# ethnhe/FFB6D

Measured on AMD Instinct MI355X. Metric: RGB-D frames/sec fwd (480x640, N=12288, bs=8), higher is better.
Workload: dtype f32; 1 GPU; FFB6D forward incl. on-device 22-call KNN index pyramid; bs=8/GPU, N=12288 pts, 480x640 RGB-D, 22 classes, fp32, eval; global_batch=8, n_points=12288, index_dtype=int64, layout=pm, parallelism=dp1 (independent batches, one process per GPU, no process group)

## Files before the change

### ffb6d_amd/csrc/mfma_pm.h

```cpp
#pragma once
#include <hip/hip_runtime.h>

namespace ffb6d {
namespace pm {

typedef float f32x16 __attribute__((ext_vector_type(16)));
typedef unsigned int u32x4 __attribute__((ext_vector_type(4)));
typedef __bf16 bf16x8 __attribute__((ext_vector_type(8)));

constexpr int BLK = 256;

template <typename T> struct El;
template <> struct El<float> {
    static constexpr int SZ = 4;
    typedef float4 Raw4;
    static __device__ __forceinline__ Raw4 ld4raw(const float* p) { return *reinterpret_cast<const float4*>(p); }
    static __device__ __forceinline__ float4 cvt4(Raw4 r) { return r; }
    static __device__ __forceinline__ float4 ld4(const float* p) { return *reinterpret_cast<const float4*>(p); }
    static __device__ __forceinline__ void st4(float* p, float4 v) { *reinterpret_cast<float4*>(p) = v; }
    static __device__ __forceinline__ float ld(const float* p) { return *p; }
    static __device__ __forceinline__ void st(float* p, float v) { *p = v; }
};
template <> struct El<__bf16> {
    static constexpr int SZ = 2;
    typedef uint2 Raw4;
    static __device__ __forceinline__ Raw4 ld4raw(const __bf16* p) { return *reinterpret_cast<const uint2*>(p); }
    static __device__ __forceinline__ float4 cvt4(Raw4 u)
    {
        return make_float4(__uint_as_float(u.x << 16), __uint_as_float(u.x & 0xffff0000u), __uint_as_float(u.y << 16),
                           __uint_as_float(u.y & 0xffff0000u));
    }
    static __device__ __forceinline__ float4 ld4(const __bf16* p) { return cvt4(ld4raw(p)); }
    static __device__ __forceinline__ void st4(__bf16* p, float4 v)
    {
        typedef __bf16 bf16x4 __attribute__((ext_vector_type(4)));
        const bf16x4 b = {(__bf16)v.x, (__bf16)v.y, (__bf16)v.z, (__bf16)v.w};
        *reinterpret_cast<bf16x4*>(p) = b;
    }
    static __device__ __forceinline__ float ld(const __bf16* p) { return (float)*p; }
    static __device__ __forceinline__ void st(__bf16* p, float v) { *p = (__bf16)v; }
};

template <typename T, int TM, int TN>
__device__ __forceinline__ void mfma_step(f32x16 (&acc)[TM][TN], const u32x4 (&a)[TM], const u32x4 (&b)[TN])
{
    if constexpr (El<T>::SZ == 4) {
#pragma unroll
        for (int tt = 0; tt < 4; ++tt)
#pragma unroll
            for (int i = 0; i < TM; ++i)
#pragma unroll
                for (int j = 0; j < TN; ++j)
                    acc[i][j] = __builtin_amdgcn_mfma_f32_32x32x2f32(__uint_as_float(a[i][tt]), __uint_as_float(b[j][tt]),
                                                                     acc[i][j], 0, 0, 0);
    } else {
#pragma unroll
        for (int i = 0; i < TM; ++i)
#pragma unroll
            for (int j = 0; j < TN; ++j)
                acc[i][j] = __builtin_amdgcn_mfma_f32_32x32x16_bf16(__builtin_bit_cast(bf16x8, a[i]), __builtin_bit_cast(bf16x8, b[j]),
                                                                    acc[i][j], 0, 0, 0);
    }
}

typedef float f32x4 __attribute__((ext_vector_type(4)));
__device__ __forceinline__ f32x4 mfma_16x16x4(float a, float b, f32x4 c)
{
#if __has_builtin(__builtin_amdgcn_mfma_f32_16x16x4f32)
    return __builtin_amdgcn_mfma_f32_16x16x4f32(a, b, c, 0, 0, 0);
#else
    const int l = (int)(threadIdx.x & 63u);
    for (int k = 0; k < 4; ++k) {
        const float bk = __shfl(b, 16 * k + (l & 15), 64);
        for (int r = 0; r < 4; ++r) c[r] = fmaf(__shfl(a, 16 * k + 4 * (l >> 4) + r, 64), bk, c[r]);
    }
    return c;
#endif
}

__device__ __forceinline__ float activate(float v, float slope) { return fmaxf(v, slope * v); }

__device__ __forceinline__ __amdgpu_buffer_rsrc_t make_rsrc(const void* base, unsigned bytes)
{
    return __builtin_amdgcn_make_buffer_rsrc(const_cast<void*>(base), 0, bytes, 0x00020000);
}

__device__ __forceinline__ void lds_dma16(__amdgpu_buffer_rsrc_t rs, unsigned char* lds_dst, int voffset, int soffset)
{
    __builtin_amdgcn_raw_ptr_buffer_load_lds(rs, (__attribute__((address_space(3))) void*)lds_dst, 16, voffset, soffset, 0, 0);
}

template <int N>
__device__ __forceinline__ void lds_dma_wait()
{
    static_assert(N >= 0 && N < 64, "vmcnt is a 6-bit counter");
#if defined(__HIP_DEVICE_COMPILE__)
    __builtin_amdgcn_s_waitcnt((N & 15) | ((N >> 4) << 14) | 0x0F70);
#endif
}

__device__ __forceinline__ int opaque(int v)
{
#if defined(__HIP_DEVICE_COMPILE__)
    asm volatile("" : "+v"(v));
#endif
    return v;
}

__device__ __forceinline__ void use_here(unsigned v)
{
#if defined(__HIP_DEVICE_COMPILE__)
    asm volatile("" ::"v"(v));
#else
    (void)v;
#endif
}

}
}
```

### ffb6d_amd/csrc/mlp_pm_split.hip

```cpp
#include <algorithm>

#include "common.h"
#include "ffb6d_ops.h"
#include "mlp_pm_common.h"

namespace ffb6d {
namespace pm {
namespace {

constexpr int SP_BLK = 512;
constexpr int SP_RB = 64;
constexpr int SP_WIMG = 256 * SP_RB;
constexpr int SP_XIMG = 128 * SP_RB;
constexpr int SP_XBASE = 3 * SP_WIMG;
constexpr int SP_STAGE = 3 * SP_WIMG + 3 * SP_XIMG;
constexpr int SP_LDS = 2 * SP_STAGE;
static_assert(SP_LDS <= 160 * 1024, "LDS layout");

typedef __bf16 bf16x2 __attribute__((ext_vector_type(2)));

__device__ __forceinline__ void split3(float a, __bf16& a0, __bf16& a1, __bf16& a2)
{
    a0 = (__bf16)a;
    const float r1 = a - (float)a0;
    a1 = (__bf16)r1;
    a2 = (__bf16)(r1 - (float)a1);
}

__global__ void __launch_bounds__(256) split_w_kernel(const float* __restrict__ w, __bf16* __restrict__ w3, long long n)
{
    for (long long e = blockIdx.x * 256LL + threadIdx.x; e < n; e += 256LL * gridDim.x) {
        __bf16 a0, a1, a2;
        split3(w[e], a0, a1, a2);
        w3[e] = a0;
        w3[n + e] = a1;
        w3[2 * n + e] = a2;
    }
}

template <int VAR>
__global__ void __launch_bounds__(SP_BLK)
mlp_pm_split_kernel(const PmParams p, const unsigned part_bytes)
{
    constexpr int OOB = 0x7ffffff0;
    extern __shared__ __attribute__((aligned(16))) unsigned char lds[];

    const int t = blockIdx.x;
    const int xcd = t & 7, sl = t >> 3;
    const int pt = (sl / p.n_ct) * 8 + xcd;
    const int ct = sl % p.n_ct;
    if (pt >= p.n_pt) return;
    const int r0 = pt * 128, c0 = ct * 256;

    const int lane = threadIdx.x & 63;
    const int l31 = lane & 31, kh = lane >> 5;
    const int wave = __builtin_amdgcn_readfirstlane(threadIdx.x >> 6);
    const int wm = wave >> 2, wn = wave & 3;
    const int K = p.k1;
    const int nstep = K / 32;
    const int wrow0 = p.rows_per_w ? (r0 / p.rows_per_w) * p.cout : 0;

    const unsigned char* w3 = static_cast<const unsigned char*>(p.w);
    const __amdgpu_buffer_rsrc_t rs_w[3] = {make_rsrc(w3, part_bytes), make_rsrc(w3 + part_bytes, part_bytes),
                                            make_rsrc(w3 + 2 * (size_t)part_bytes, part_bytes)};
    const __amdgpu_buffer_rsrc_t rs_x = make_rsrc(p.x1, span_bytes((unsigned)p.rows, p.ld1, p.k1, 4));

    const int lrow = 16 * wave + (lane >> 2);
    const int lchunk = ((lane & 3) ^ ((lrow >> 3) & 3)) * 16;
    int w_off[2];
#pragma unroll
    for (int h = 0; h < 2; ++h) {
        const int ch = c0 + 128 * h + lrow;
        w_off[h] = ch < p.cout ? (wrow0 + ch) * (K * 2) + lchunk : OOB;
    }
    auto request_w = [&](int s, int stage) {
        unsigned char* wi = lds + stage * SP_STAGE + wave * (16 * SP_RB);
#pragma unroll
        for (int pi = 0; pi < 3; ++pi)
#pragma unroll
            for (int h = 0; h < 2; ++h) lds_dma16(rs_w[pi], wi + pi * SP_WIMG + h * (128 * SP_RB), w_off[h], s * SP_RB);
    };

    const int xrow = threadIdx.x >> 2, xq = threadIdx.x & 3;
    const bool xlive = r0 + xrow < p.rows;
    const int x_off0 = xlive ? (r0 + xrow) * p.ld1 * 4 + xq * 32 : OOB;
    const int x_off1 = xlive ? x_off0 + 16 : OOB;
    const int x_dst = SP_XBASE + xrow * SP_RB + ((xq ^ ((xrow >> 3) & 3)) * 16);
    auto load_x = [&](int s, u32x4 (&v)[2]) {
        v[0] = __builtin_amdgcn_raw_buffer_load_b128(rs_x, x_off0, s * 128, 0);
        v[1] = __builtin_amdgcn_raw_buffer_load_b128(rs_x, x_off1, s * 128, 0);
    };
    auto write_x = [&](int stage, const u32x4 (&v)[2]) {
        u32x4 o[3];
        if constexpr (VAR & 1) {
#pragma unroll
            for (int q = 0; q < 4; ++q) {
                const unsigned pk = (v[q >> 1][2 * (q & 1)] >> 16) | (v[q >> 1][2 * (q & 1) + 1] & 0xffff0000u);
                o[0][q] = pk; o[1][q] = 0u; o[2][q] = 0u;
            }
        } else {
#pragma unroll
            for (int q = 0; q < 4; ++q) {
                bf16x2 b0, b1, b2;
                __bf16 s0, s1, s2;
                split3(__uint_as_float(v[q >> 1][2 * (q & 1)]), s0, s1, s2);
                b0[0] = s0; b1[0] = s1; b2[0] = s2;
                split3(__uint_as_float(v[q >> 1][2 * (q & 1) + 1]), s0, s1, s2);
                b0[1] = s0; b1[1] = s1; b2[1] = s2;
                o[0][q] = __builtin_bit_cast(unsigned, b0);
                o[1][q] = __builtin_bit_cast(unsigned, b1);
                o[2][q] = __builtin_bit_cast(unsigned, b2);
            }
        }
        unsigned char* xi = lds + stage * SP_STAGE + x_dst;
#pragma unroll
        for (int pj = 0; pj < 3; ++pj) *reinterpret_cast<u32x4*>(xi + pj * SP_XIMG) = o[pj];
    };

    const int fsw = (l31 >> 3) & 3;
    const int a_row = (wm * 128 + l31) * SP_RB, b_row = SP_XBASE + (wn * 32 + l31) * SP_RB;
    f32x16 acc[4][1];
#pragma unroll
    for (int i = 0; i < 4; ++i)
#pragma unroll
        for (int r = 0; r < 16; ++r) acc[i][0][r] = 0.f;

    auto multiply = [&](int stage, int ks) {
        const unsigned char* im = lds + stage * SP_STAGE;
        const int fo = ((2 * ks + kh) ^ fsw) * 16;
        u32x4 a[3][4], b[3];
#pragma unroll
        for (int pj = 0; pj < 3; ++pj) b[pj] = *reinterpret_cast<const u32x4*>(im + b_row + pj * SP_XIMG + fo);
#pragma unroll
        for (int pi = 0; pi < 3; ++pi)
#pragma unroll
            for (int i = 0; i < 4; ++i) a[pi][i] = *reinterpret_cast<const u32x4*>(im + pi * SP_WIMG + a_row + i * (32 * SP_RB) + fo);
        if constexpr (VAR & 2) {
#pragma unroll
            for (int pi = 0; pi < 3; ++pi)
#pragma unroll
                for (int i = 0; i < 4; ++i) use_here(a[pi][i][0] ^ b[pi][3]);
            return;
        }
        constexpr int TW[6] = {0, 1, 2, 0, 1, 0}, TX[6] = {2, 1, 0, 1, 0, 0};
#pragma unroll
        for (int tm = 0; tm < 6; ++tm)
#pragma unroll
            for (int i = 0; i < 4; ++i)
                acc[i][0] = __builtin_amdgcn_mfma_f32_32x32x16_bf16(__builtin_bit_cast(bf16x8, a[TW[tm]][i]),
                                                                   __builtin_bit_cast(bf16x8, b[TX[tm]]), acc[i][0], 0, 0, 0);
    };

    {
        u32x4 xv[2];
        request_w(0, 0);
        load_x(0, xv);
        write_x(0, xv);
    }
    __syncthreads();
    for (int s = 0; s < nstep; ++s) {
        const int st = s & 1;
        const bool more = s + 1 < nstep;
        u32x4 xv[2];
        if (more) {
            request_w(s + 1, st ^ 1);
            load_x(s + 1, xv);
        }
        __builtin_amdgcn_sched_barrier(0);
        multiply(st, 0);
        __builtin_amdgcn_sched_barrier(0);
        if (more) write_x(st ^ 1, xv);
        __builtin_amdgcn_sched_barrier(0);
        multiply(st, 1);
        __builtin_amdgcn_sched_barrier(0);
        lds_dma_wait<0>();
        __syncthreads();
    }
    if constexpr (VAR & 4) {
        if (p.act != 77) return;
    }
    pm_epilogue<float, 4, 1, false>(p, acc, c0, r0, wm, wn, l31, kh);
}

template <int VAR>
bool launch_split(PmParams& p, unsigned part_bytes, hipStream_t st)
{
    static int attr_set[kMaxDevices + 1];
    const int slot = device_slot();
    if (!cache_get(attr_set, slot)) {
        if (hipFuncSetAttribute(reinterpret_cast<const void*>(&mlp_pm_split_kernel<VAR>), hipFuncAttributeMaxDynamicSharedMemorySize, SP_LDS) !=
            hipSuccess)
            return false;
        cache_set(attr_set, slot, 1);
    }
    p.n_ct = (int)ceil_div(p.cout, 256);
    p.n_pt = (int)ceil_div(p.rows, 128);
    const unsigned grid = (unsigned)(ceil_div(p.n_pt, 8) * 8 * p.n_ct);
    hipLaunchKernelGGL(mlp_pm_split_kernel<VAR>, dim3(grid), dim3(SP_BLK), SP_LDS, st, p, part_bytes);
    return true;
}

bool split_form_ok(const PmParams& p, int64_t w_rows, int64_t y_rows)
{
    const int64_t K = p.k1;
    return p.k2 == 0 && !p.x2 && !p.xidx && p.act >= 0 && p.act <= 2 && K % 32 == 0 && K >= 64 && (p.cout & 3) == 0 &&
           (p.ld1 & 3) == 0 && ((reinterpret_cast<uintptr_t>(p.x1) | reinterpret_cast<uintptr_t>(p.w)) & 15) == 0 &&
           ((int64_t)p.rows + 256) * p.ld1 * 4 < (1LL << 31) && ((int64_t)p.rows + 256) * p.ldo * 4 < (1LL << 31) &&
           (w_rows + 256) * K * 2 < (1LL << 31) && (!p.y || (y_rows + 256) * p.ldy * 4 < (1LL << 31));
}

}
}
}

using namespace ffb6d;
using namespace ffb6d::pm;

extern "C" int ffb6d_mlp_pm_split_w(const float* w, void* w3, int64_t n, ffb6d_stream_t stream)
{
    FFB6D_REQUIRE(n >= 0, "mlp_pm_split_w: bad size");
    if (n == 0) return FFB6D_OK;
    FFB6D_REQUIRE(w && w3, "mlp_pm_split_w: null pointer");
    const unsigned grid = (unsigned)std::min<int64_t>(ceil_div(n, 256), 4096);
    hipLaunchKernelGGL(split_w_kernel, dim3(grid), dim3(256), 0, as_stream(stream), w, static_cast<__bf16*>(w3), (long long)n);
    FFB6D_LAUNCH_CHECK();
    return FFB6D_OK;
}

extern "C" int ffb6d_mlp_pm_split_f32(const void* w3, const float* bias, const float* x1, int64_t k1, int64_t ld1, const void* x1_idx,
                                      int64_t x1_rows_per_frame, const float* x2, int64_t k2, int64_t ld2, const float* y, int64_t ldy,
                                      const void* y_idx, int64_t y_rows_per_frame, int idx_bits, int64_t rows_per_frame, float* out,
                                      int64_t ldo, int64_t rows, int64_t cout, int act, int variant, ffb6d_stream_t stream)
{
    (void)x1_rows_per_frame; (void)ld2;
    FFB6D_REQUIRE(rows >= 0 && cout >= 1 && k1 >= 1 && k2 >= 0, "mlp_pm_split: bad shape");
#ifndef FFB6D_SPLIT_PROBES
    FFB6D_REQUIRE(variant == 0, "mlp_pm_split: the library carries variant 0 only");
#endif
    if (rows == 0) return FFB6D_OK;
    FFB6D_REQUIRE(w3 && x1 && out, "mlp_pm_split: null pointer");
    FFB6D_REQUIRE(ld1 >= k1 && ldo >= cout, "mlp_pm_split: row stride smaller than the row");
    FFB6D_REQUIRE(!y_idx || y, "mlp_pm_split: gather indices without rows to gather");
    FFB6D_REQUIRE(!y_idx || ((idx_bits == 32 || idx_bits == 64) && rows_per_frame >= 1 && rows % rows_per_frame == 0 && y_rows_per_frame >= 1),
                  "mlp_pm_split: index arrays need idx_bits 32/64 and rows_per_frame dividing rows");
    FFB6D_REQUIRE(!y || ldy >= cout, "mlp_pm_split: ldy smaller than cout");
    PmParams p;
    p.w = w3; p.bias = bias; p.x1 = x1; p.xidx = x1_idx; p.x2 = x2; p.y = y; p.gidx = y_idx; p.out = out;
    p.rows = (int)rows; p.cout = (int)cout; p.k1 = (int)k1; p.k2 = (int)k2; p.ld1 = (int)ld1; p.ld2 = 4;
    p.ldy = (int)ldy; p.ldo = (int)ldo; p.P = (int)(y_idx ? rows_per_frame : rows); p.py = (int)y_rows_per_frame; p.px = 0;
    p.act = act; p.idx64 = idx_bits == 64;
    const int64_t y_rows = y ? (y_idx ? rows / rows_per_frame * y_rows_per_frame : rows) : 0;
    FFB6D_REQUIRE(rows < (1LL << 31) && cout < (1LL << 31) && k1 < (1LL << 31) && ld1 < (1LL << 31) && ldo < (1LL << 31) && ldy < (1LL << 31) &&
                  split_form_ok(p, cout, y_rows),
                  "mlp_pm_split: the split-bf16 form needs one ungathered fp32 source with K %% 32 == 0, K >= 64, cout %% 4 == 0, "
                  "16-byte aligned operand rows, act 0..2 and buffers under 2 GiB");
    const unsigned part_bytes = (unsigned)(cout * k1 * 2);
    bool ok;
    switch (variant) {
#ifdef FFB6D_SPLIT_PROBES
        case 1: ok = launch_split<1>(p, part_bytes, as_stream(stream)); break;
        case 2: ok = launch_split<2>(p, part_bytes, as_stream(stream)); break;
        case 4: ok = launch_split<4>(p, part_bytes, as_stream(stream)); break;
        case 6: ok = launch_split<6>(p, part_bytes, as_stream(stream)); break;
#endif
        default: ok = launch_split<0>(p, part_bytes, as_stream(stream)); break;
    }
    if (!ok)
        return set_error(FFB6D_ERR_HIP, "mlp_pm_split: hipFuncSetAttribute(MaxDynamicSharedMemorySize) failed");
    FFB6D_LAUNCH_CHECK();
    return FFB6D_OK;
}

extern "C" int ffb6d_mlp_pm_split_batched_f32(const void* w3, int64_t n_w, int64_t rows_per_w, const float* x, int64_t k, int64_t ld,
                                              float* out, int64_t ldo, int64_t rows, int64_t cout, ffb6d_stream_t stream)
{
    FFB6D_REQUIRE(rows >= 0 && cout >= 1 && k >= 1 && n_w >= 1, "mlp_pm_split_batched: bad shape");
    FFB6D_REQUIRE(rows_per_w >= 128 && rows_per_w % 128 == 0 && rows_per_w < (1LL << 31),
                  "mlp_pm_split_batched: rows_per_w must be a positive multiple of 128 (got %lld): a point tile multiplies one matrix",
                  (long long)rows_per_w);
    if (rows == 0) return FFB6D_OK;
    FFB6D_REQUIRE(w3 && x && out, "mlp_pm_split_batched: null pointer");
    FFB6D_REQUIRE(ld >= k && ldo >= cout && ceil_div(rows, rows_per_w) <= n_w, "mlp_pm_split_batched: stride smaller than the row, or more "
                  "rows than matrices");
    PmParams p;
    p.w = w3; p.bias = nullptr; p.x1 = x; p.xidx = nullptr; p.x2 = nullptr; p.y = nullptr; p.gidx = nullptr; p.out = out;
    p.rows = (int)rows; p.cout = (int)cout; p.k1 = (int)k; p.k2 = 0; p.ld1 = (int)ld; p.ld2 = 4; p.ldy = 0; p.ldo = (int)ldo;
    p.P = (int)rows; p.py = 0; p.px = 0; p.act = 0; p.idx64 = 0;
    p.rows_per_w = (int)rows_per_w; p.w_stride = (int)(cout * k);
    FFB6D_REQUIRE(rows < (1LL << 31) && cout < (1LL << 31) && k < (1LL << 31) && ld < (1LL << 31) && ldo < (1LL << 31) &&
                  n_w * cout < (1LL << 31) && split_form_ok(p, n_w * cout, 0),
                  "mlp_pm_split_batched: needs K %% 32 == 0, K >= 64, cout %% 4 == 0, 16-byte aligned rows and buffers under 2 GiB");
    if (!launch_split<0>(p, (unsigned)(n_w * cout * k * 2), as_stream(stream)))
        return set_error(FFB6D_ERR_HIP, "mlp_pm_split_batched: hipFuncSetAttribute(MaxDynamicSharedMemorySize) failed");
    FFB6D_LAUNCH_CHECK();
    return FFB6D_OK;
}
```

Measured before the change: 729.5 frames/s.

## Software-pipeline split-bf16 MLP GEMM with interleaved DMA, fragment loads and MFMA

Restructures the main loop of the split-bf16 pointwise MLP kernel into a ring-slot pipeline. Weight LDS-DMA requests, next-k-step fragment reads and x split/stores are interleaved between individual MFMA groups using sched barriers and group barriers. It also issues x global loads two slots ahead and replaces the full waitcnt plus __syncthreads with a partial vmcnt ring_wait and a raw s_barrier. The goal is to hide global/LDS latency behind matrix ops, at the cost of more registers (double fragment sets) and fragile manual scheduling.

```diff
diff --git a/ffb6d_amd/csrc/mfma_pm.h b/ffb6d_amd/csrc/mfma_pm.h
--- a/ffb6d_amd/csrc/mfma_pm.h
+++ b/ffb6d_amd/csrc/mfma_pm.h
@@ -99,6 +99,15 @@
 #endif
 }
 
+template <int N>
+__device__ __forceinline__ void ring_wait()
+{
+    static_assert(N >= 0 && N < 64, "vmcnt is a 6-bit counter");
+#if defined(__HIP_DEVICE_COMPILE__)
+    __builtin_amdgcn_s_waitcnt((N & 15) | ((N >> 4) << 14) | 0x0070);
+#endif
+}
+
 __device__ __forceinline__ int opaque(int v)
 {
 #if defined(__HIP_DEVICE_COMPILE__)
diff --git a/ffb6d_amd/csrc/mlp_pm_split.hip b/ffb6d_amd/csrc/mlp_pm_split.hip
--- a/ffb6d_amd/csrc/mlp_pm_split.hip
+++ b/ffb6d_amd/csrc/mlp_pm_split.hip
@@ -1,4 +1,5 @@
 #include <algorithm>
+#include <type_traits>
 
 #include "common.h"
 #include "ffb6d_ops.h"
@@ -9,13 +10,18 @@
 namespace {
 
 constexpr int SP_BLK = 512;
-constexpr int SP_RB = 64;
+constexpr int SP_KS = 32;
+constexpr int SP_RB = 2 * SP_KS;
 constexpr int SP_WIMG = 256 * SP_RB;
 constexpr int SP_XIMG = 128 * SP_RB;
 constexpr int SP_XBASE = 3 * SP_WIMG;
-constexpr int SP_STAGE = 3 * SP_WIMG + 3 * SP_XIMG;
-constexpr int SP_LDS = 2 * SP_STAGE;
+constexpr int SP_SLOT = 3 * SP_WIMG + 3 * SP_XIMG;
+constexpr int SP_NS = 2;
+constexpr int SP_LDS = SP_NS * SP_SLOT;
 static_assert(SP_LDS <= 160 * 1024, "LDS layout");
+constexpr int SP_NW = 6;
+constexpr int SP_NV = 2;
+constexpr int SP_NOP = SP_NW + SP_NV;
 
 typedef __bf16 bf16x2 __attribute__((ext_vector_type(2)));
 
@@ -57,7 +63,7 @@
     const int wave = __builtin_amdgcn_readfirstlane(threadIdx.x >> 6);
     const int wm = wave >> 2, wn = wave & 3;
     const int K = p.k1;
-    const int nstep = K / 32;
+    const int nslot = K / SP_KS;
     const int wrow0 = p.rows_per_w ? (r0 / p.rows_per_w) * p.cout : 0;
 
     const unsigned char* w3 = static_cast<const unsigned char*>(p.w);
@@ -73,48 +79,56 @@
         const int ch = c0 + 128 * h + lrow;
         w_off[h] = ch < p.cout ? (wrow0 + ch) * (K * 2) + lchunk : OOB;
     }
-    auto request_w = [&](int s, int stage) {
-        unsigned char* wi = lds + stage * SP_STAGE + wave * (16 * SP_RB);
+    auto request_w = [&](int j, int rs, int q0 = 0, int q1 = SP_NW) {
+        const bool in = j < nslot;
+        const int so = in ? j * SP_RB : 0;
+        unsigned char* wi = lds + rs * SP_SLOT + wave * (16 * SP_RB);
 #pragma unroll
         for (int pi = 0; pi < 3; ++pi)
 #pragma unroll
-            for (int h = 0; h < 2; ++h) lds_dma16(rs_w[pi], wi + pi * SP_WIMG + h * (128 * SP_RB), w_off[h], s * SP_RB);
+            for (int h = 0; h < 2; ++h)
+                if (pi * 2 + h >= q0 && pi * 2 + h < q1)
+                    lds_dma16(rs_w[pi], wi + pi * SP_WIMG + h * (128 * SP_RB), in ? w_off[h] : OOB, so);
     };
 
     const int xrow = threadIdx.x >> 2, xq = threadIdx.x & 3;
     const bool xlive = r0 + xrow < p.rows;
-    const int x_off0 = xlive ? (r0 + xrow) * p.ld1 * 4 + xq * 32 : OOB;
-    const int x_off1 = xlive ? x_off0 + 16 : OOB;
+    int x_off[SP_NV];
+#pragma unroll
+    for (int q = 0; q < SP_NV; ++q) x_off[q] = xlive ? (r0 + xrow) * p.ld1 * 4 + xq * 32 + 16 * q : OOB;
     const int x_dst = SP_XBASE + xrow * SP_RB + ((xq ^ ((xrow >> 3) & 3)) * 16);
-    auto load_x = [&](int s, u32x4 (&v)[2]) {
-        v[0] = __builtin_amdgcn_raw_buffer_load_b128(rs_x, x_off0, s * 128, 0);
-        v[1] = __builtin_amdgcn_raw_buffer_load_b128(rs_x, x_off1, s * 128, 0);
-    };
-    auto write_x = [&](int stage, const u32x4 (&v)[2]) {
-        u32x4 o[3];
+    auto load_x = [&](int j, u32x4 (&v)[SP_NV]) {
+        const bool in = j < nslot;
+        const int so = in ? j * (SP_KS * 4) : 0;
+#pragma unroll
+        for (int q = 0; q < SP_NV; ++q) v[q] = __builtin_amdgcn_raw_buffer_load_b128(rs_x, in ? x_off[q] : OOB, so, 0);
+    };
+    auto split_pair = [&](const u32x4 (&v)[SP_NV], int q, unsigned (&o)[3][4]) {
         if constexpr (VAR & 1) {
-#pragma unroll
-            for (int q = 0; q < 4; ++q) {
-                const unsigned pk = (v[q >> 1][2 * (q & 1)] >> 16) | (v[q >> 1][2 * (q & 1) + 1] & 0xffff0000u);
-                o[0][q] = pk; o[1][q] = 0u; o[2][q] = 0u;
-            }
+            o[0][q] = (v[q >> 1][2 * (q & 1)] >> 16) | (v[q >> 1][2 * (q & 1) + 1] & 0xffff0000u);
+            o[1][q] = 0u; o[2][q] = 0u;
         } else {
-#pragma unroll
-            for (int q = 0; q < 4; ++q) {
-                bf16x2 b0, b1, b2;
-                __bf16 s0, s1, s2;
-                split3(__uint_as_float(v[q >> 1][2 * (q & 1)]), s0, s1, s2);
-                b0[0] = s0; b1[0] = s1; b2[0] = s2;
-                split3(__uint_as_float(v[q >> 1][2 * (q & 1) + 1]), s0, s1, s2);
-                b0[1] = s0; b1[1] = s1; b2[1] = s2;
-                o[0][q] = __builtin_bit_cast(unsigned, b0);
-                o[1][q] = __builtin_bit_cast(unsigned, b1);
-                o[2][q] = __builtin_bit_cast(unsigned, b2);
-            }
-        }
-        unsigned char* xi = lds + stage * SP_STAGE + x_dst;
-#pragma unroll
-        for (int pj = 0; pj < 3; ++pj) *reinterpret_cast<u32x4*>(xi + pj * SP_XIMG) = o[pj];
+            bf16x2 b0, b1, b2;
+            __bf16 s0, s1, s2;
+            split3(__uint_as_float(v[q >> 1][2 * (q & 1)]), s0, s1, s2);
+            b0[0] = s0; b1[0] = s1; b2[0] = s2;
+            split3(__uint_as_float(v[q >> 1][2 * (q & 1) + 1]), s0, s1, s2);
+            b0[1] = s0; b1[1] = s1; b2[1] = s2;
+            o[0][q] = __builtin_bit_cast(unsigned, b0);
+            o[1][q] = __builtin_bit_cast(unsigned, b1);
+            o[2][q] = __builtin_bit_cast(unsigned, b2);
+        }
+    };
+    auto store_x = [&](int rs, const unsigned (&o)[3][4]) {
+        unsigned char* xi = lds + rs * SP_SLOT + x_dst;
+#pragma unroll
+        for (int pj = 0; pj < 3; ++pj) *reinterpret_cast<u32x4*>(xi + pj * SP_XIMG) = u32x4{o[pj][0], o[pj][1], o[pj][2], o[pj][3]};
+    };
+    auto write_x = [&](int rs, const u32x4 (&v)[SP_NV]) {
+        unsigned o[3][4];
+#pragma unroll
+        for (int q = 0; q < 4; ++q) split_pair(v, q, o);
+        store_x(rs, o);
     };
 
     const int fsw = (l31 >> 3) & 3;
@@ -125,57 +139,102 @@
 #pragma unroll
         for (int r = 0; r < 16; ++r) acc[i][0][r] = 0.f;
 
-    auto multiply = [&](int stage, int ks) {
-        const unsigned char* im = lds + stage * SP_STAGE;
+    auto frags = [&](int rs, int ks, u32x4 (&a)[3][4], u32x4 (&b)[3], int q0 = 0, int q1 = 15) {
+        const unsigned char* im = lds + rs * SP_SLOT;
         const int fo = ((2 * ks + kh) ^ fsw) * 16;
-        u32x4 a[3][4], b[3];
-#pragma unroll
-        for (int pj = 0; pj < 3; ++pj) b[pj] = *reinterpret_cast<const u32x4*>(im + b_row + pj * SP_XIMG + fo);
-#pragma unroll
-        for (int pi = 0; pi < 3; ++pi)
-#pragma unroll
-            for (int i = 0; i < 4; ++i) a[pi][i] = *reinterpret_cast<const u32x4*>(im + pi * SP_WIMG + a_row + i * (32 * SP_RB) + fo);
+#pragma unroll
+        for (int g = 0; g < 3; ++g) {
+            if (5 * g >= q0 && 5 * g < q1) b[2 - g] = *reinterpret_cast<const u32x4*>(im + b_row + (2 - g) * SP_XIMG + fo);
+#pragma unroll
+            for (int i = 0; i < 4; ++i)
+                if (5 * g + 1 + i >= q0 && 5 * g + 1 + i < q1)
+                    a[g][i] = *reinterpret_cast<const u32x4*>(im + g * SP_WIMG + a_row + i * (32 * SP_RB) + fo);
+        }
+    };
+    auto mma = [&](const u32x4 (&a)[3][4], const u32x4 (&b)[3], int t0, int t1) {
         if constexpr (VAR & 2) {
-#pragma unroll
-            for (int pi = 0; pi < 3; ++pi)
-#pragma unroll
-                for (int i = 0; i < 4; ++i) use_here(a[pi][i][0] ^ b[pi][3]);
+            if (t0 == 0) {
+#pragma unroll
+                for (int pi = 0; pi < 3; ++pi)
+#pragma unroll
+                    for (int i = 0; i < 4; ++i) use_here(a[pi][i][0] ^ b[pi][3]);
+            }
             return;
         }
         constexpr int TW[6] = {0, 1, 2, 0, 1, 0}, TX[6] = {2, 1, 0, 1, 0, 0};
 #pragma unroll
-        for (int tm = 0; tm < 6; ++tm)
+        for (int tm = 0; tm < 6; ++tm) {
+            if (tm < t0 || tm >= t1) continue;
 #pragma unroll
             for (int i = 0; i < 4; ++i)
                 acc[i][0] = __builtin_amdgcn_mfma_f32_32x32x16_bf16(__builtin_bit_cast(bf16x8, a[TW[tm]][i]),
                                                                    __builtin_bit_cast(bf16x8, b[TX[tm]]), acc[i][0], 0, 0, 0);
-    };
-
-    {
-        u32x4 xv[2];
-        request_w(0, 0);
-        load_x(0, xv);
-        write_x(0, xv);
-    }
-    __syncthreads();
-    for (int s = 0; s < nstep; ++s) {
-        const int st = s & 1;
-        const bool more = s + 1 < nstep;
-        u32x4 xv[2];
-        if (more) {
-            request_w(s + 1, st ^ 1);
-            load_x(s + 1, xv);
-        }
-        __builtin_amdgcn_sched_barrier(0);
-        multiply(st, 0);
-        __builtin_amdgcn_sched_barrier(0);
-        if (more) write_x(st ^ 1, xv);
-        __builtin_amdgcn_sched_barrier(0);
-        multiply(st, 1);
-        __builtin_amdgcn_sched_barrier(0);
-        lds_dma_wait<0>();
-        __syncthreads();
-    }
+        }
+    };
+
+    constexpr int WAIT_X = (SP_NS - 1) * SP_NOP, WAIT_W = SP_NV + (SP_NS - 2) * SP_NOP;
+    u32x4 xr[SP_NS][SP_NV];
+    load_x(0, xr[0]);
+#pragma unroll
+    for (int j = 0; j < SP_NS - 1; ++j) {
+        __builtin_amdgcn_sched_barrier(0);
+        request_w(j, j);
+        __builtin_amdgcn_sched_barrier(0);
+        load_x(j + 1, xr[j + 1]);
+    }
+    __builtin_amdgcn_sched_barrier(0);
+    write_x(0, xr[0]);
+    __builtin_amdgcn_sched_barrier(0);
+    ring_wait<SP_NV>();
+    __builtin_amdgcn_s_barrier();
+    __builtin_amdgcn_sched_barrier(0);
+    auto iteration = [&](int h, auto uc) {
+        constexpr int u = decltype(uc)::value;
+        u32x4 a[2][3][4], b[2][3];
+        frags(u, 0, a[0], b[0], 0, 5);
+        __builtin_amdgcn_sched_barrier(0);
+        frags(u, 0, a[0], b[0], 5, 10);
+        __builtin_amdgcn_sched_barrier(0);
+        frags(u, 0, a[0], b[0], 10, 15);
+#pragma unroll
+        for (int tm = 0; tm < 6; ++tm) {
+            __builtin_amdgcn_sched_barrier(0);
+            mma(a[0], b[0], tm, tm + 1);
+            __builtin_amdgcn_sched_barrier(0);
+            request_w(h + SP_NS - 1, (u + SP_NS - 1) % SP_NS, tm, tm + 1);
+            frags(u, 1, a[1], b[1], tm < 3 ? 3 * tm : 9 + 2 * (tm - 3), tm < 3 ? 3 * tm + 3 : 11 + 2 * (tm - 3));
+        }
+        __builtin_amdgcn_sched_barrier(0);
+        load_x(h + SP_NS, xr[u]);
+        __builtin_amdgcn_sched_barrier(0);
+        lds_dma_wait<WAIT_X>();
+        unsigned o[3][4];
+#pragma unroll
+        for (int tm = 0; tm < 6; ++tm) {
+            __builtin_amdgcn_sched_barrier(0);
+            mma(a[1], b[1], tm, tm + 1);
+            if (tm < 4) {
+                split_pair(xr[(u + 1) % SP_NS], tm, o);
+#pragma unroll
+                for (int i = 0; i < 4; ++i) {
+                    __builtin_amdgcn_sched_group_barrier(0x008, 1, 0);
+                    __builtin_amdgcn_sched_group_barrier(0x002, 5, 0);
+                }
+            }
+            if (tm == 4) store_x((u + 1) % SP_NS, o);
+        }
+        __builtin_amdgcn_sched_barrier(0);
+        ring_wait<WAIT_W>();
+        __builtin_amdgcn_s_barrier();
+        __builtin_amdgcn_sched_barrier(0);
+    };
+    int h0 = 0;
+    for (; h0 + SP_NS <= nslot; h0 += SP_NS) {
+        iteration(h0, std::integral_constant<int, 0>());
+        iteration(h0 + 1, std::integral_constant<int, 1>());
+    }
+    if (h0 < nslot) iteration(h0, std::integral_constant<int, 0>());
+    lds_dma_wait<0>();
     if constexpr (VAR & 4) {
         if (p.act != 77) return;
     }
```

Result: faster. 751.2 frames/s (median of 6 runs) (+3.0%).
